# MasterBin-IIAU/Unicorn

Hardware: NVIDIA H100
Metric: frames/sec (higher is better)
Workload: dtype bf16

## Files before the change

### unicorn_b200/csrc/dwconv_mma.cu

```cuda
#include "uc_ptx.cuh"
#include "uc_common.h"
#include "../../include/unicorn_b200.h"
#include <algorithm>

namespace uc {

constexpr int kMmTW = 16, kMmTH = 16, kMmCH = 32;
constexpr int kMmHW = kMmTW + 8, kMmHH = kMmTH + 6;
constexpr int kMmPixBytes = kMmCH * 2;
constexpr int kMmStageBytes = kMmHH * kMmHW * kMmPixBytes;
constexpr int kMmPlaneBytes = kMmHH * kMmHW * 2;
constexpr int kMmPlanarBytes = kMmCH * kMmPlaneBytes;
constexpr int kMmPairBytes = kMmCH * 7 * 8 * 4;
constexpr int kMmQBytes = kMmPairBytes + kMmCH * 4;
constexpr int kMmSmem = kMmStageBytes + kMmPlanarBytes + kMmQBytes + 128 + 128;
constexpr int kMmWarps = 4, kMmCtasPerSm = 3;

struct alignas(64) DwMmaParams {
  CUtensorMap tmX;
  const uint8_t* qtab;
  uint16_t* y;
  int* work_counter;
  int H, W, C, B, tiles_w, tiles_h, n_items;
};

__device__ __forceinline__ int mm_plane(int c) { return (c & 7) * 4 + (c >> 3); }

__device__ __forceinline__ void bulk_load_1d(void* smem, const void* gmem, uint32_t bytes, uint64_t* bar) {
  asm volatile("cp.async.bulk.shared::cluster.global.mbarrier::complete_tx::bytes [%0], [%1], %2, [%3];" ::"r"(smem_u32(smem)), "l"(gmem),
               "r"(bytes), "r"(smem_u32(bar))
               : "memory");
}

struct DwFrag {
  uint32_t a[2][6];
  uint32_t q[2];
};

__global__ void __launch_bounds__(kMmWarps * 32, kMmCtasPerSm) dwconv7_mma_kernel(const __grid_constant__ DwMmaParams p) {
  constexpr int CPW = kMmCH / kMmWarps;
  extern __shared__ uint8_t dsm_raw[];
  uint8_t* stage = dsm_raw + ((128u - (smem_u32(dsm_raw) & 127u)) & 127u);
  uint8_t* planar = stage + kMmStageBytes;
  uint8_t* qs = planar + kMmPlanarBytes;
  uint64_t* bar = reinterpret_cast<uint64_t*>(qs + kMmQBytes);
  volatile int* s_info = reinterpret_cast<volatile int*>(bar + 2);
  const int lane = threadIdx.x & 31, warp = threadIdx.x >> 5;
  const int g = lane >> 2, t = lane & 3;
  if (threadIdx.x == 0) {
    prefetch_tmap(&p.tmX);
    mbar_init(&bar[0], 1);
    mbar_init(&bar[1], 1);
    fence_barrier_init();
  }
  __syncthreads();
  pdl_wait();
  pdl_launch_dependents();
  const int tiles_img = p.tiles_w * p.tiles_h, tiles_chunk = tiles_img * p.B;
  int static_next = blockIdx.x;
  auto fetch = [&]() {
    if (p.work_counter) return atomicAdd(p.work_counter, 1);
    const int item = static_next;
    static_next += gridDim.x;
    return item;
  };
  auto issue = [&](int slot, int item) {
    volatile int* info = s_info + slot * 4;
    if (item >= p.n_items) {
      info[0] = -1;
      mbar_arrive(&bar[0]);
      return;
    }
    const int chunk = item / tiles_chunk, tt0 = item - chunk * tiles_chunk;
    const int b = tt0 / tiles_img, tt = tt0 - b * tiles_img;
    const int oh0 = (tt / p.tiles_w) * kMmTH, ow0 = (tt % p.tiles_w) * kMmTW;
    info[0] = chunk; info[1] = b; info[2] = oh0; info[3] = ow0;
    mbar_arrive_expect_tx(&bar[0], kMmStageBytes);
    tma_load_4d(stage, &p.tmX, &bar[0], chunk * kMmCH, ow0 - 4, oh0 - 3, b);
  };
  int pending = 0;
  if (threadIdx.x == 0) {
    issue(0, fetch());
    pending = fetch();
  }
  const int fc = warp * CPW;
  const uint32_t planar_w = smem_u32(planar) + mm_plane(fc) * kMmPlaneBytes;
  const uint32_t lm4 = planar_w + static_cast<uint32_t>((((lane & 7) + ((lane >> 3) & 1) * 8) * kMmHW + (lane >> 4) * 8) * 2);
  const uint32_t lm2 = planar_w + static_cast<uint32_t>(((lane & 15) * kMmHW + 16) * 2);
  const int d = 2 * t - g - 1;
  const bool first = d >= -1;
  const uint32_t q_lane = smem_u32(qs) + static_cast<uint32_t>((fc * 7 * 8 + (first ? d + 1 : d + 9)) * 4);
  const float* bias_s = reinterpret_cast<const float*>(qs + kMmPairBytes) + fc;
  const int tq = lane & 3, tsw = (lane >> 2) & 1;
  const uint32_t sel_lo = tsw ? 0x1054u : 0x5410u, sel_hi = tsw ? 0x3276u : 0x7632u;
  auto load_frag = [&](int s, DwFrag& f) {
    const int kh = s % 7;
#pragma unroll
    for (int j = 0; j < 2; ++j) {
      const int c = (s / 7) * 2 + j;
      const uint32_t off = static_cast<uint32_t>(c * 4 * kMmPlaneBytes + kh * (kMmHW * 2));
      asm volatile("ldmatrix.sync.aligned.m8n8.x4.shared.b16 {%0,%1,%2,%3}, [%4];"
                   : "=r"(f.a[j][0]), "=r"(f.a[j][1]), "=r"(f.a[j][2]), "=r"(f.a[j][3]) : "r"(lm4 + off));
      asm volatile("ldmatrix.sync.aligned.m8n8.x2.shared.b16 {%0,%1}, [%2];" : "=r"(f.a[j][4]), "=r"(f.a[j][5]) : "r"(lm2 + off));
      asm volatile("ld.shared.b32 %0, [%1];" : "=r"(f.q[j]) : "r"(q_lane + static_cast<uint32_t>((c * 7 + kh) * 32)));
    }
  };
  int prev_chunk = -1;
  uint32_t q_phase = 0;
  for (int it = 0;; ++it) {
    mbar_wait(&bar[0], it & 1);
    const int chunk = s_info[(it & 1) * 4 + 0];
    if (chunk < 0) break;
    const int b = s_info[(it & 1) * 4 + 1], oh0 = s_info[(it & 1) * 4 + 2], ow0 = s_info[(it & 1) * 4 + 3];
    const int c0 = chunk * kMmCH + fc;
    const bool new_chunk = chunk != prev_chunk;
    prev_chunk = chunk;
    if (new_chunk && threadIdx.x == 0) {
      mbar_arrive_expect_tx(&bar[1], kMmQBytes);
      bulk_load_1d(qs, p.qtab + static_cast<size_t>(chunk) * kMmQBytes, kMmQBytes, &bar[1]);
    }
    {
      const uint4* st = reinterpret_cast<const uint4*>(stage);
#pragma unroll 3
      for (int pp = warp * 8 + (lane >> 2); pp < kMmHH * kMmHW / 2; pp += kMmWarps * 8) {
        const uint4 va = st[(2 * pp + tsw) * 4 + tq];
        const uint4 vb = st[(2 * pp + (tsw ^ 1)) * 4 + tq];
        const uint32_t wa[4] = {va.x, va.y, va.z, va.w}, wb[4] = {vb.x, vb.y, vb.z, vb.w};
        uint8_t* dst = planar + pp * 4;
#pragma unroll
        for (int j = 0; j < 8; ++j)
          *reinterpret_cast<uint32_t*>(dst + mm_plane(tq * 8 + j) * kMmPlaneBytes) = __byte_perm(wa[j >> 1], wb[j >> 1], j & 1 ? sel_hi : sel_lo);
      }
    }
    __syncthreads();
    if (threadIdx.x == 0) {
      issue((it + 1) & 1, pending);
      pending = fetch();
    }
    if (new_chunk) {
      mbar_wait(&bar[1], q_phase);
      q_phase ^= 1;
    }
    if (c0 < p.C) {
      float acc[CPW][2][4];
#pragma unroll
      for (int c = 0; c < CPW; ++c) {
        const float bv = bias_s[c];
#pragma unroll
        for (int e = 0; e < 4; ++e) acc[c][0][e] = acc[c][1][e] = bv;
      }
      DwFrag fr[2];
      load_frag(0, fr[0]);
#pragma unroll
      for (int s = 0; s < CPW / 2 * 7; ++s) {
        if (s + 1 < CPW / 2 * 7) load_frag(s + 1, fr[(s + 1) & 1]);
        const DwFrag& f = fr[s & 1];
#pragma unroll
        for (int j = 0; j < 2; ++j) {
          const int c = (s / 7) * 2 + j;
          const uint32_t b0 = first ? f.q[j] : 0u, b1 = first ? 0u : f.q[j];
#pragma unroll
          for (int nb = 0; nb < 2; ++nb)
            asm volatile("mma.sync.aligned.m16n8k16.row.col.f32.bf16.bf16.f32 {%0,%1,%2,%3}, {%4,%5,%6,%7}, {%8,%9}, {%0,%1,%2,%3};"
                         : "+f"(acc[c][nb][0]), "+f"(acc[c][nb][1]), "+f"(acc[c][nb][2]), "+f"(acc[c][nb][3])
                         : "r"(f.a[j][2 * nb]), "r"(f.a[j][2 * nb + 1]), "r"(f.a[j][2 * nb + 2]), "r"(f.a[j][2 * nb + 3]), "r"(b0), "r"(b1));
        }
      }
      uint16_t* yb = p.y + ((static_cast<size_t>(b) * p.H + oh0) * p.W + ow0) * p.C + c0;
#pragma unroll
      for (int nb = 0; nb < 2; ++nb)
#pragma unroll
        for (int e = 0; e < 4; ++e) {
          const int r = g + (e >> 1) * 8, cl = nb * 8 + 2 * t + (e & 1);
          if (oh0 + r < p.H && ow0 + cl < p.W) {
            uint4 o;
            o.x = pack_bf16(acc[0][nb][e], acc[1][nb][e]); o.y = pack_bf16(acc[2][nb][e], acc[3][nb][e]);
            o.z = pack_bf16(acc[4][nb][e], acc[5][nb][e]); o.w = pack_bf16(acc[6][nb][e], acc[7][nb][e]);
            *reinterpret_cast<uint4*>(yb + (static_cast<size_t>(r) * p.W + cl) * p.C) = o;
          }
        }
    }
    __syncthreads();
  }
}

}

using namespace uc;

extern "C" int uc_dwconv7_mma(const void* x_bf16, const void* qtab, void* y_bf16, int B, int H, int W, int C,
                              int* work_counter, void* stream_v) {
  cudaStream_t stream = static_cast<cudaStream_t>(stream_v);
  if (!x_bf16 || !qtab || !y_bf16) return set_error(UC_EINVAL, "uc_dwconv7_mma: null pointer");
  if (x_bf16 == y_bf16) return set_error(UC_EINVAL, "uc_dwconv7_mma: not an in-place operation");
  if (B < 1 || H < 1 || W < 1 || C < 8 || C % 8) return set_error(UC_EINVAL, "uc_dwconv7_mma: C must be a multiple of 8");
  if ((reinterpret_cast<uintptr_t>(x_bf16) | reinterpret_cast<uintptr_t>(y_bf16) | reinterpret_cast<uintptr_t>(qtab)) & 15) return set_error(UC_EINVAL, "uc_dwconv7_mma: 16-byte aligned maps");
  int rc = ensure_driver();
  if (rc) return rc;
  DwMmaParams p;
  memset(&p, 0, sizeof(p));
  {
    uint64_t dims[4] = {static_cast<uint64_t>(C), static_cast<uint64_t>(W), static_cast<uint64_t>(H), static_cast<uint64_t>(B)};
    uint64_t strides[3] = {static_cast<uint64_t>(C) * 2, static_cast<uint64_t>(W) * C * 2, static_cast<uint64_t>(H) * W * C * 2};
    uint32_t box[4] = {kMmCH, kMmHW, kMmHH, 1};
    rc = encode_tmap(&p.tmX, CU_TENSOR_MAP_DATA_TYPE_BFLOAT16, 4, x_bf16, dims, strides, box, CU_TENSOR_MAP_SWIZZLE_NONE);
    if (rc) return rc;
  }
  p.qtab = static_cast<const uint8_t*>(qtab);
  p.y = static_cast<uint16_t*>(y_bf16);
  p.work_counter = work_counter;
  p.H = H; p.W = W; p.C = C; p.B = B;
  p.tiles_w = (W + kMmTW - 1) / kMmTW;
  p.tiles_h = (H + kMmTH - 1) / kMmTH;
  const long items = static_cast<long>(p.tiles_w) * p.tiles_h * B * ((C + kMmCH - 1) / kMmCH);
  if (items > 0x7fffffffL) return set_error(UC_EINVAL, "uc_dwconv7_mma: too many tiles");
  p.n_items = static_cast<int>(items);
  static PerDeviceFlag attr_dev;
  bool& attr = attr_dev.get();
  if (!attr) {
    cudaError_t e = cudaFuncSetAttribute(dwconv7_mma_kernel, cudaFuncAttributeMaxDynamicSharedMemorySize, kMmSmem);
    if (e != cudaSuccess) return set_error(static_cast<int>(e), "uc_dwconv7_mma: cudaFuncSetAttribute: %s", cudaGetErrorString(e));
    attr = true;
  }
  const int grid = static_cast<int>(std::min<long>(items, static_cast<long>(num_sms()) * kMmCtasPerSm));
  cudaError_t e = launch_pdl(dwconv7_mma_kernel, dim3(grid), dim3(kMmWarps * 32), kMmSmem, stream, p);
  if (e != cudaSuccess) return set_error(static_cast<int>(e), "uc_dwconv7_mma launch: %s", cudaGetErrorString(e));
  return check_launch("uc_dwconv7_mma");
}
```

Measured before the change: 182.6.

## Stage depthwise-conv output tile in swizzled smem and write with TMA store

Instead of each thread issuing scattered 16-byte global stores with bounds checks, the accumulators are packed into a 64B-swizzled shared-memory tile, reusing the planar buffer, and stored with a single TMA tensor store per tile. TMA clips out-of-bounds rows and columns, which removes the per-element bounds checks. The cost is extra __syncthreads barriers, a proxy fence, and a wait-for-read on the store before the buffer is reused, which serialises part of the loop. Each store also carries a risk if the 512-aligned tile offset inside the planar region does not fit.

```diff
diff --git a/unicorn_b200/csrc/dwconv_mma.cu b/unicorn_b200/csrc/dwconv_mma.cu
--- a/unicorn_b200/csrc/dwconv_mma.cu
+++ b/unicorn_b200/csrc/dwconv_mma.cu
@@ -18,8 +18,8 @@
 
 struct alignas(64) DwMmaParams {
   CUtensorMap tmX;
+  CUtensorMap tmY;
   const uint8_t* qtab;
-  uint16_t* y;
   int* work_counter;
   int H, W, C, B, tiles_w, tiles_h, n_items;
 };
@@ -49,6 +49,7 @@
   const int g = lane >> 2, t = lane & 3;
   if (threadIdx.x == 0) {
     prefetch_tmap(&p.tmX);
+    prefetch_tmap(&p.tmY);
     mbar_init(&bar[0], 1);
     mbar_init(&bar[1], 1);
     fence_barrier_init();
@@ -110,7 +111,10 @@
   for (int it = 0;; ++it) {
     mbar_wait(&bar[0], it & 1);
     const int chunk = s_info[(it & 1) * 4 + 0];
-    if (chunk < 0) break;
+    if (chunk < 0) {
+      if (threadIdx.x == 0) tma_store_wait_all();
+      break;
+    }
     const int b = s_info[(it & 1) * 4 + 1], oh0 = s_info[(it & 1) * 4 + 2], ow0 = s_info[(it & 1) * 4 + 3];
     const int c0 = chunk * kMmCH + fc;
     const bool new_chunk = chunk != prev_chunk;
@@ -141,8 +145,9 @@
       mbar_wait(&bar[1], q_phase);
       q_phase ^= 1;
     }
-    if (c0 < p.C) {
-      float acc[CPW][2][4];
+    const bool active = c0 < p.C;
+    float acc[CPW][2][4];
+    if (active) {
 #pragma unroll
       for (int c = 0; c < CPW; ++c) {
         const float bv = bias_s[c];
@@ -166,19 +171,28 @@
                          : "r"(f.a[j][2 * nb]), "r"(f.a[j][2 * nb + 1]), "r"(f.a[j][2 * nb + 2]), "r"(f.a[j][2 * nb + 3]), "r"(b0), "r"(b1));
         }
       }
-      uint16_t* yb = p.y + ((static_cast<size_t>(b) * p.H + oh0) * p.W + ow0) * p.C + c0;
+    }
+    __syncthreads();
+    uint8_t* tile = planar + ((512u - (smem_u32(planar) & 511u)) & 511u);
+    if (active) {
 #pragma unroll
       for (int nb = 0; nb < 2; ++nb)
 #pragma unroll
         for (int e = 0; e < 4; ++e) {
           const int r = g + (e >> 1) * 8, cl = nb * 8 + 2 * t + (e & 1);
-          if (oh0 + r < p.H && ow0 + cl < p.W) {
-            uint4 o;
-            o.x = pack_bf16(acc[0][nb][e], acc[1][nb][e]); o.y = pack_bf16(acc[2][nb][e], acc[3][nb][e]);
-            o.z = pack_bf16(acc[4][nb][e], acc[5][nb][e]); o.w = pack_bf16(acc[6][nb][e], acc[7][nb][e]);
-            *reinterpret_cast<uint4*>(yb + (static_cast<size_t>(r) * p.W + cl) * p.C) = o;
-          }
+          uint4 o;
+          o.x = pack_bf16(acc[0][nb][e], acc[1][nb][e]); o.y = pack_bf16(acc[2][nb][e], acc[3][nb][e]);
+          o.z = pack_bf16(acc[4][nb][e], acc[5][nb][e]); o.w = pack_bf16(acc[6][nb][e], acc[7][nb][e]);
+          const uint32_t off = (r * kMmTW + cl) * 64 + warp * 16;
+          *reinterpret_cast<uint4*>(tile + (off ^ (((off >> 7) & 3) << 4))) = o;
         }
+    }
+    fence_proxy_async();
+    __syncthreads();
+    if (threadIdx.x == 0) {
+      tma_store_4d(&p.tmY, tile, chunk * kMmCH, ow0, oh0, b);
+      tma_store_commit();
+      tma_store_wait_read();
     }
     __syncthreads();
   }
@@ -205,9 +219,11 @@
     uint32_t box[4] = {kMmCH, kMmHW, kMmHH, 1};
     rc = encode_tmap(&p.tmX, CU_TENSOR_MAP_DATA_TYPE_BFLOAT16, 4, x_bf16, dims, strides, box, CU_TENSOR_MAP_SWIZZLE_NONE);
     if (rc) return rc;
+    uint32_t ybox[4] = {kMmCH, kMmTW, kMmTH, 1};
+    rc = encode_tmap(&p.tmY, CU_TENSOR_MAP_DATA_TYPE_BFLOAT16, 4, y_bf16, dims, strides, ybox, CU_TENSOR_MAP_SWIZZLE_64B);
+    if (rc) return rc;
   }
   p.qtab = static_cast<const uint8_t*>(qtab);
-  p.y = static_cast<uint16_t*>(y_bf16);
   p.work_counter = work_counter;
   p.H = H; p.W = W; p.C = C; p.B = B;
   p.tiles_w = (W + kMmTW - 1) / kMmTW;
```

New measurement: 186.0 (median of 6 runs). 1.9% higher.
